# nverchev/PointCloudCounterfactual

Hardware: AMD Instinct MI355X
Metric: clouds/sec Chamfer+EMD fwd+bwd, N=2048 B=32 (higher is better)
Workload: dtype f32; 1 GPU; BASELINE configs[1]+[2]: N=2048 B=32 per GPU, nn_distance (Chamfer, mean) fwd+bwd + match_cost (approxmatch+matchcost) fwd+bwd through the autograd surface; inputs = "recon" clouds (reference permuted + N(0, 0.02^2): a trained autoencoder, SURVEY 8(d)); the 8(d) stress set (both clouds i.i.d. U[0,1]^3) is value_stress (--full); emd_mode=implicit, batch_per_gpu=32, n_points=2048, global_batch=32, parallelism=batch-sharded x1, no data-path collective, launcher=single process

## Files before the change

### include/pcc_test_hooks.h

```cpp
#ifndef PCC_TEST_HOOKS_H
#define PCC_TEST_HOOKS_H

#ifdef __cplusplus
extern "C" {
#endif
#pragma GCC visibility push(default)

int pcc_test_inject_auction_failure(void);
int pcc_test_inject_approxmatch_failure(void);

enum {
    PCC_TUNE_AM_NOCULL = 2,
    PCC_TUNE_AM_NOSPLIT = 3,
    PCC_TUNE_AM_NORESIDENT = 4,
    PCC_TUNE_EDGE_SCATTER = 5,
    PCC_TUNE_NBRSUM_SCATTER = 6,
    PCC_TUNE_AUCTION_CLUSTER = 7,
    PCC_TUNE_KNN_NOSPLIT = 8,
    PCC_TUNE_KNN_WIDE = 9
};
int pcc_test_set_tuning(int key, int value);

#pragma GCC visibility pop
#ifdef __cplusplus
}
#endif
#endif
```

### pointcloudcounterfactual_amd/_lib.py

```python

from __future__ import annotations

import ctypes
import os
from typing import Any

import torch

_HERE = os.path.dirname(os.path.abspath(__file__))
LIB_PATH = os.environ.get('PCC_LIB_OVERRIDE') or os.path.join(_HERE, 'lib', 'libpcc_structural.so')

_vp = ctypes.c_void_p
_int = ctypes.c_int

ABI: dict[str, tuple[object, list[object]]] = {
    'pcc_version': (ctypes.c_char_p, []),
    'pcc_last_error': (ctypes.c_char_p, []),
    'pcc_last_status': (_int, []),
    'pcc_profile_enable': (None, [_int]),
    'pcc_profile_reset': (None, []),
    'pcc_profile_read': (_int, [ctypes.c_char_p, ctypes.POINTER(ctypes.c_double), ctypes.POINTER(ctypes.c_int)]),
    'nndistance': (None, [_int, _int, _vp, _int, _vp, _vp, _vp, _vp, _vp, _vp]),
    'pcc_nndistance': (_int, [_int, _int, _vp, _int, _vp, _vp, _vp, _vp, _vp, _vp]),
    'nndistancegrad': (None, [_int, _int, _vp, _int, _vp, _vp, _vp, _vp, _vp, _vp, _vp, _vp]),
# ... 32 lines not shown
    'pcc_bn_relu_bwd': (_int, [_int, _int, _int, _vp, _vp, _vp, ctypes.c_float, _vp, _vp, _vp, _int, _vp, _vp, _vp, _vp]),
    'pcc_auction_forward': (_int, [_int, _int, _vp, _vp, ctypes.c_float, _int, _vp, _vp, _vp]),
    'pcc_auction_status': (_int, []),
    'pcc_auction_backward': (_int, [_int, _int, _vp, _vp, _vp, _vp, _vp, _vp]),
    'pcc_test_inject_auction_failure': (_int, []),
    'pcc_test_inject_approxmatch_failure': (_int, []),
    'pcc_test_set_tuning': (_int, [_int, _int]),
}


def _load() -> ctypes.CDLL:
    if not os.path.exists(LIB_PATH):
        raise ImportError(
            f'{LIB_PATH} is missing: the HIP extension has not been built '
            '(run `make -C pointcloudcounterfactual_amd/csrc`); there is no fallback path.'
        )
    lib = ctypes.CDLL(LIB_PATH)
    for name, (restype, argtypes) in ABI.items():
        fn = getattr(lib, name)
        fn.restype = restype
        fn.argtypes = argtypes
    return lib


lib = _load()


def check(status: int, what: str) -> None:
    if status != 0:
        msg = lib.pcc_last_error().decode() or f'HIP kernel failed : {status}'
        raise RuntimeError(f'{what}: {msg}')


def ptr(t: torch.Tensor | None, name: str, dtype: torch.dtype, device: torch.device) -> int | None:
    if t is None:
        return None
    if t.device != device or device.type != 'cuda':
        if t.device.type != 'cuda':
            raise RuntimeError(f'{name} must be a CUDA tensor')
        raise RuntimeError(f'{name} is on {t.device}, expected {device}')
    if not t.is_contiguous():
        raise RuntimeError(f'{name} must be contiguous')
    if t.dtype != dtype:
        raise RuntimeError(f'{name} must be {dtype}, found {t.dtype}')
    return t.data_ptr()


def call(fn: Any, what: str, device: torch.device, *args: Any) -> None:
    with torch.cuda.device(device):
        check(fn(*args, torch.cuda.current_stream(device).cuda_stream), what)


TUNING = {'am_nocull': 2, 'am_nosplit': 3, 'am_noresident': 4, 'edge_scatter': 5, 'nbrsum_scatter': 6,
          'auction_cluster': 7, 'knn_nosplit': 8, 'knn_wide': 9}


def set_tuning(name: str, value: int) -> None:
    if lib.pcc_test_set_tuning(TUNING[name], int(value)) != 1:
        raise RuntimeError('test hooks are not armed: set PCC_TEST_HOOKS=1 before the library is loaded')
```

### pointcloudcounterfactual_amd/csrc/approxmatch.hip

```cpp
#include "pcc_common.hpp"
#include "pcc_test_hooks.h"
#include "wave_sort.hpp"

#include <algorithm>
#include <functional>
#include <mutex>
#include <type_traits>

namespace {

using pcc::sq3;

typedef float v4f __attribute__((ext_vector_type(4)));

constexpr int kLevels = 9;
constexpr float kLog2e = 1.44269504088896340736f;

struct LevelConsts {
    float c[kLevels];
};

__host__ LevelConsts make_levels() {
    LevelConsts lc;
    float level = -16384.0f;
    for (int i = 0; i < kLevels; i++) {
        lc.c[i] = level * kLog2e;
        level *= 0.25f;
    }
    return lc;
}

__device__ __forceinline__ float fast_exp2(float x) { return __builtin_amdgcn_exp2f(x); }

enum Phase { PH_A = 0, PH_B = 1, PH_CA = 2, PH_C = 3 };

__device__ __forceinline__ float pass_a_ratio(float remL, float sum) { return remL / (1e-9f + sum); }
struct PassB {
    float ratio, remain;
};
__device__ __forceinline__ PassB pass_b(float remR, float sum) {
    const float sumr = sum * remR;
    const float consumption = __builtin_fminf(remR / (sumr + 1e-9f), 1.0f);
    return {consumption * remR, __builtin_fmaxf(0.0f, remR - sumr)};
}
__device__ __forceinline__ float pass_c_left(float remL, float ratioL, float sum) { return __builtin_fmaxf(0.0f, remL - ratioL * sum); }

constexpr int kBox = 16;
constexpr int kLiveRow = 16;
constexpr int kInfSlot = 13;
constexpr float kZeroExp = 151.f;

struct PhaseArgs {
    int n_own, n_cand, tiles, batch;
    int own_n4, cand_n4, own_nb, cand_nb;
    const float *own_soa, *cand_soa;
    const float *cand_box;
    const float *own_box16;
    const float *w0, *w1;
    long long w0_stride, w1_stride;
    float w0c;
    float c0, c1;
// ... 366 lines not shown
                const unsigned long long alive = __ballot(remain_new != 0.f);
                if (lane == 0) atomicAdd(&a.live_out[(size_t)smp * kLiveRow], (int)__popcll(alive));
            }
            if (COWN && a.mask_out && remain_new == 0.f)
                atomicAnd(&a.mask_out[(size_t)smp * kLevels * a.mask_words + (o >> 5)], ~(1u << (o & 31)));
            if (COWN && a.clist) {
                float cx = ox[0], cy = oy[0], cz = oz[0];
#pragma unroll
                for (int r = 1; r < R; r++) {
                    cx = w == r ? ox[r] : cx;
                    cy = w == r ? oy[r] : cy;
                    cz = w == r ? oz[r] : cz;
                }
                float *cl = a.clist + (size_t)smp * 5 * a.cl_n4 + tile * TQ + e;
                cl[0] = cx;
                cl[(size_t)a.cl_n4] = cy;
                cl[(size_t)2 * a.cl_n4] = cz;
                cl[(size_t)3 * a.cl_n4] = ratio_new;
                cl[(size_t)4 * a.cl_n4] = remain_new;
            }
        } else {
            const float left = pass_c_left(a.first ? a.multiL : pre_rem, pre_ratio, t0);
            a.remain[(size_t)smp * a.remain_stride + o] = left;
            if (MODE == PH_CA) a.ratio_out[(size_t)smp * a.ratio_stride + o] = pass_a_ratio(left, t1);
        }
    }
}


template <int MODE, int R, int S, int CH, int VAR, int G = 1>
__global__ __launch_bounds__(64 * S) void am_phase_kernel(PhaseArgs a) {
    __shared__ __attribute__((aligned(16))) float smem[PhaseLds<(MODE == PH_CA ? 2 : 1), R, S, CH>::floats];
    constexpr bool COWN = VAR == V_COWN;
    int smp, tile;
    const int bid = (int)blockIdx.x, nwg = (int)gridDim.x;
    if (COWN) {
        if (a.batch % 8 == 0) {
            const int per = a.batch / 8, i = bid / 8;
            smp = (bid % 8) + 8 * (i % per);
            tile = i / per;
        } else {
            smp = bid % a.batch;
            tile = bid / a.batch;
        }
        if (a.live_in && tile > 0 && tile * (64 * R / G) >= a.live_in[(size_t)smp * kLiveRow]) return;
    } else {
        const int lid = pcc::xcd_contiguous(bid, nwg);
        smp = lid / a.tiles;
        tile = lid - smp * a.tiles;
    }
    am_phase_body<MODE, R, S, CH, VAR, G>(a, smp, tile, smem);
}

constexpr int kFineS = 8;
constexpr int kFineOG = 16;
constexpr int kFineGroups = 64 / kFineOG;
constexpr int kFineQ = 4;

__device__ __forceinline__ float row_sum16(float v) {
    v += __int_as_float(__builtin_amdgcn_update_dpp(0, __float_as_int(v), 0xB1, 0xF, 0xF, true));
    v += __int_as_float(__builtin_amdgcn_update_dpp(0, __float_as_int(v), 0x4E, 0xF, 0xF, true));
    v += __int_as_float(__builtin_amdgcn_update_dpp(0, __float_as_int(v), 0x141, 0xF, 0xF, true));
    v += __int_as_float(__builtin_amdgcn_update_dpp(0, __float_as_int(v), 0x140, 0xF, 0xF, true));
    return v;
}

struct FineOwners {
    float x[kFineQ], y[kFineQ], z[kFineQ];
};
struct FineRows {
    const float *x, *y, *z, *w0, *w1;
};

__device__ __forceinline__ void fine_group_box(const float *own_box, int own_nb, int smp, int g16, float4 &lo, float4 &hi) {
    lo = make_float4(__builtin_inff(), __builtin_inff(), __builtin_inff(), 0.f);
    hi = make_float4(-__builtin_inff(), -__builtin_inff(), -__builtin_inff(), 0.f);
    if (g16 < own_nb) {
        const float4 *ob = reinterpret_cast<const float4 *>(own_box + ((size_t)smp * own_nb + g16) * 8);
        lo = ob[0];
        hi = ob[1];
    }
}

__device__ __forceinline__ float fine_box_d2(const float4 &glo, const float4 &ghi, const float *cand_box) {
    const float4 *cb = reinterpret_cast<const float4 *>(cand_box);
    const float4 lo = cb[0], hi = cb[1];
    const float dx = fmaxf(fmaxf(glo.x - hi.x, lo.x - ghi.x), 0.f);
    const float dy = fmaxf(fmaxf(glo.y - hi.y, lo.y - ghi.y), 0.f);
    const float dz = fmaxf(fmaxf(glo.z - hi.z, lo.z - ghi.z), 0.f);
    return dx * dx + dy * dy + dz * dz;
}

template <int NBLK>
__device__ __forceinline__ void fine_block_list(bool keep, bool outer_only, int tid, int tg, int tb, int w, int lane,
                                                int *wave_cnt, unsigned char (*items)[NBLK], unsigned char *need) {
    if (tid < NBLK) need[tid] = 0;
    const unsigned long long bal = __ballot(keep);
    if (lane == 0) wave_cnt[w] = __popcll(bal);
    __syncthreads();
    const int before = (w & 1) ? wave_cnt[w - 1] : 0;
    if (keep) {
        items[tg][before + __popcll(bal & ((1ull << lane) - 1ull))] = (unsigned char)(tb | (outer_only ? 128 : 0));
        need[tb] = 1;
    }
    __syncthreads();
}

template <int NW>
__device__ __forceinline__ void fine_walk(const FineRows &rows, const unsigned char *list, int nitems, int cs, int cl, float c0,
                                          float c1, const FineOwners &own, float (&s0)[kFineQ], float (&s1)[kFineQ]) {
    for (int it = cs; it < nitems; it += 2) {
        const int item = __builtin_amdgcn_readfirstlane((int)list[it]);
        const int ci = (item & 127) * kBox + cl;
        const float x = rows.x[ci], y = rows.y[ci], z = rows.z[ci];
        if (NW == 2 && (item & 128)) {
            const float wb = rows.w1[ci];
#pragma unroll
            for (int j = 0; j < kFineQ; j++) s1[j] = __builtin_fmaf(fast_exp2(c1 * sq3(x - own.x[j], y - own.y[j], z - own.z[j])), wb, s1[j]);
            continue;
        }
        const float wa = rows.w0[ci];
        float wb = 0.f;
        if (NW == 2) wb = rows.w1[ci];
#pragma unroll
        for (int j = 0; j < kFineQ; j++) {
            const float d = sq3(x - own.x[j], y - own.y[j], z - own.z[j]);
            s0[j] = __builtin_fmaf(fast_exp2(c0 * d), wa, s0[j]);
            if (NW == 2) s1[j] = __builtin_fmaf(fast_exp2(c1 * d), wb, s1[j]);
        }
    }
}

template <int NW>
__device__ __forceinline__ void fine_reduce(float (&s0)[kFineQ], float (&s1)[kFineQ], float (*red)[2][64], int cs, int cl, int og, int quad) {
#pragma unroll
    for (int j = 0; j < kFineQ; j++) {
        s0[j] = row_sum16(s0[j]);
        if (NW == 2) s1[j] = row_sum16(s1[j]);
    }
    if (cl == 0) {
#pragma unroll
        for (int j = 0; j < kFineQ; j++) {
            red[0][cs][og * kFineOG + quad * kFineQ + j] = s0[j];
            if (NW == 2) red[1][cs][og * kFineOG + quad * kFineQ + j] = s1[j];
        }
    }
}

template <int MODE, int CH>
__global__ __launch_bounds__(64 * kFineS, MODE == PH_CA ? 4 : 8) void am_fine_kernel(PhaseArgs a) {
    constexpr int T = 64 * kFineS;
    constexpr int NW = (MODE == PH_CA) ? 2 : 1;
    constexpr bool W0_CONST = (MODE == PH_A);
    constexpr int NBLK = CH / kBox;
    static_assert(kFineGroups * NBLK == T, "one (owner group, candidate block) box test per thread");
    static_assert(kFineOG == kBox && kFineOG * kFineQ == 64, "a wave = 16 candidates x 4 owner quads");
    __shared__ __attribute__((aligned(16))) float lds_c[(3 + NW) * CH];
    __shared__ float red[NW][2][64];
    __shared__ unsigned char items[kFineGroups][NBLK];
    __shared__ unsigned char need[NBLK];
    __shared__ int wave_cnt[kFineS];

    const int lid = pcc::xcd_contiguous((int)blockIdx.x, (int)gridDim.x);
    const int smp = lid / a.tiles;
    const int tile = lid - smp * a.tiles;
    const int tid = threadIdx.x, lane = tid & 63;
    const int w = __builtin_amdgcn_readfirstlane(tid >> 6);
    const int og = w & (kFineGroups - 1);
    const int cs = w / kFineGroups;
    const int cl = lane & (kBox - 1);
    const int quad = lane / kBox;
    const float *O = a.own_soa + (size_t)smp * 3 * a.own_n4;
    const float *C = a.cand_soa + (size_t)smp * 3 * a.cand_n4;
    const float *W0 = W0_CONST ? nullptr : a.w0 + (size_t)smp * a.w0_stride;
    const float *W1 = (NW == 2) ? a.w1 + (size_t)smp * a.w1_stride : nullptr;

    FineOwners own;
    float s0[kFineQ], s1[kFineQ];
#pragma unroll
    for (int j = 0; j < kFineQ; j++) {
        int o = tile * 64 + og * kFineOG + quad * kFineQ + j;
        o = o < a.n_own ? o : a.n_own - 1;
        own.x[j] = O[o];
        own.y[j] = O[a.own_n4 + o];
        own.z[j] = O[2 * a.own_n4 + o];
        s0[j] = 0.f;
        s1[j] = 0.f;
    }
    const int own_e = (tid < 64 && tile * 64 + tid < a.n_own) ? tile * 64 + tid : -1;
    float pre_rem = 0.f, pre_ratio = 0.f;
    {
        const int oe = max(own_e, 0);
        if (MODE != PH_A && !a.first) pre_rem = a.remain[(size_t)smp * a.remain_stride + oe];
        if (MODE == PH_CA || MODE == PH_C) pre_ratio = a.ratio_in[(size_t)smp * a.ratio_stride + oe];
    }
    const int tg = tid / NBLK, tb = tid - tg * NBLK;
    float4 glo, ghi;
    fine_group_box(a.own_box16, a.own_nb, smp, tile * kFineGroups + tg, glo, ghi);
    const float c0 = a.c0, c1 = a.c1, cut2 = a.cut2;
    const FineRows rows = {lds_c, lds_c + CH, lds_c + 2 * CH, lds_c + 3 * CH, lds_c + 4 * CH};

    for (int q0 = 0; q0 < a.n_cand; q0 += CH) {
        const int cnt = min(CH, a.n_cand - q0);
        const int ngroups = (cnt + 3) / 4;
        const int nblk = (ngroups + 3) / 4;
        if (q0) __syncthreads();
        bool keep = false, outer_only = false;
        if (tb < nblk) {
            const float bd2 = fine_box_d2(glo, ghi, a.cand_box + ((size_t)smp * a.cand_nb + q0 / kBox + tb) * 8);
            keep = !(bd2 > cut2);
            outer_only = NW == 2 && bd2 > a.cut2_fine;
        }
        fine_block_list<NBLK>(keep, outer_only, tid, tg, tb, w, lane, wave_cnt, items, need);
        {
            float4 *dst4 = reinterpret_cast<float4 *>(lds_c);
            const float4 *sx = reinterpret_cast<const float4 *>(C + q0);
            const float4 *sy = reinterpret_cast<const float4 *>(C + (size_t)a.cand_n4 + q0);
            const float4 *sz = reinterpret_cast<const float4 *>(C + (size_t)2 * a.cand_n4 + q0);
            static_assert(CH / 4 <= T, "one float4 group per thread and chunk");
            const int i = tid;
            if (i < nblk * 4 && need[i >> 2]) {
                float4 vx = make_float4(0.f, 0.f, 0.f, 0.f), vy = vx, vz = vx, v0 = vx, v1 = vx;
                if (i < ngroups) {
                    vx = sx[i]; vy = sy[i]; vz = sz[i];
                    v0 = W0_CONST ? make_float4(a.w0c, a.w0c, a.w0c, a.w0c) : *reinterpret_cast<const float4 *>(W0 + q0 + 4 * i);
                    if (NW == 2) v1 = *reinterpret_cast<const float4 *>(W1 + q0 + 4 * i);
                    if (W0_CONST && i * 4 + 3 >= cnt) {
                        v0.x = i * 4 + 0 < cnt ? v0.x : 0.f;
                        v0.y = i * 4 + 1 < cnt ? v0.y : 0.f;
                        v0.z = i * 4 + 2 < cnt ? v0.z : 0.f;
                        v0.w = 0.f;
                    }
                }
                dst4[i] = vx;
                dst4[CH / 4 + i] = vy;
                dst4[2 * (CH / 4) + i] = vz;
                dst4[3 * (CH / 4) + i] = v0;
                if (NW == 2) dst4[4 * (CH / 4) + i] = v1;
            }
        }
        __syncthreads();
        fine_walk<NW>(rows, items[og], wave_cnt[2 * og] + wave_cnt[2 * og + 1], cs, cl, c0, c1, own, s0, s1);
    }
    fine_reduce<NW>(s0, s1, red, cs, cl, og, quad);
    __syncthreads();
    if (own_e < 0) return;
    const float sum0 = red[0][0][tid] + red[0][1][tid];
    const float sum1 = NW == 2 ? red[NW - 1][0][tid] + red[NW - 1][1][tid] : 0.f;
    if (MODE == PH_A) {
        a.ratio_out[(size_t)smp * a.ratio_stride + own_e] = pass_a_ratio(a.multiL, sum0);
    } else if (MODE == PH_B) {
        const PassB pb = pass_b(a.first ? a.multiR : pre_rem, sum0);
        a.ratio_out[(size_t)smp * a.ratio_stride + own_e] = pb.ratio;
        a.remain_out[(size_t)smp * a.remain_stride + own_e] = pb.remain;
        if (a.live_out) {
            const unsigned long long alive = __ballot(pb.remain != 0.f);
            if (lane == 0) atomicAdd(&a.live_out[(size_t)smp * kLiveRow], (int)__popcll(alive));
            if (a.mask_out && lane == 0) {
                unsigned *mo = a.mask_out + (size_t)smp * kLevels * a.mask_words;
                if (2 * tile < a.mask_words) mo[2 * tile] = (unsigned)alive;
                if (2 * tile + 1 < a.mask_words) mo[2 * tile + 1] = (unsigned)(alive >> 32);
            }
        }
    } else {
        const float left = pass_c_left(a.first ? a.multiL : pre_rem, pre_ratio, sum0);
        a.remain[(size_t)smp * a.remain_stride + own_e] = left;
        if (MODE == PH_CA) a.ratio_out[(size_t)smp * a.ratio_stride + own_e] = pass_a_ratio(left, sum1);
    }
}

constexpr int kFpPasses = 7;
constexpr int kFpCH = 2048;
constexpr int kBarSlot = 12;
constexpr int kErrSlot = 15;

struct FinePersistArgs {
    int n, m, n4, m4, nb1, nb2, tiles;
    const float *soa1, *soa2, *box1, *box2;
    float *rem, *lv;
    float multiL, multiR;
    float c[4], cut2[4];
    int *live_cnt;
    unsigned *live_mask;
    int mask_words;
    unsigned *host_err;
    int inject;
};

__global__ __launch_bounds__(64 * kFineS) void am_fine_persist_kernel(FinePersistArgs a) {
    constexpr int T = 64 * kFineS, CH = kFpCH, NBLK = CH / kBox;
    static_assert(kFineGroups * NBLK == T, "one (owner group, candidate block) box test per thread and direction");
    __shared__ __attribute__((aligned(16))) float lds_p[2][3 * CH];
    __shared__ __attribute__((aligned(16))) float lds_w[2][CH];
    __shared__ float red[2][2][64];
    __shared__ unsigned char items[kFineGroups][NBLK];
    __shared__ unsigned char need[NBLK];
    __shared__ int wave_cnt[kFineS];

    const int lid = pcc::xcd_contiguous((int)blockIdx.x, (int)gridDim.x);
    const int smp = lid / a.tiles;
    const int tile = lid - smp * a.tiles;
    const int tid = threadIdx.x, lane = tid & 63;
    const int w = __builtin_amdgcn_readfirstlane(tid >> 6);
    const int og = w & (kFineGroups - 1), cs = w / kFineGroups;
    const int cl = lane & (kBox - 1), quad = lane / kBox;
    const long long nm4 = (long long)a.n4 + a.m4, rs = (long long)a.n4 + 2LL * a.m4;
    const float *S1 = a.soa1 + (size_t)smp * 3 * a.n4;
    const float *S2 = a.soa2 + (size_t)smp * 3 * a.m4;
    float *LV = a.lv + (size_t)smp * kLevels * nm4;
    float *REM = a.rem + (size_t)smp * rs;
    int *row = a.live_cnt + (size_t)smp * kLiveRow;
    unsigned *bar = reinterpret_cast<unsigned *>(row + kBarSlot);
    unsigned *err = reinterpret_cast<unsigned *>(row + kErrSlot);

    for (int s = 0; s < 2; s++) {
        const float *S = s ? S2 : S1;
        const int p4 = s ? a.m4 : a.n4, ngroups = p4 / 4, nblk = (ngroups + 3) / 4;
        float4 *dst4 = reinterpret_cast<float4 *>(lds_p[s]);
        const float4 *sx = reinterpret_cast<const float4 *>(S);
        const float4 *sy = reinterpret_cast<const float4 *>(S + p4);
        const float4 *sz = reinterpret_cast<const float4 *>(S + 2 * (size_t)p4);
        for (int i = tid; i < nblk * 4; i += T) {
            float4 vx = make_float4(0.f, 0.f, 0.f, 0.f), vy = vx, vz = vx;
            if (i < ngroups) { vx = sx[i]; vy = sy[i]; vz = sz[i]; }
            dst4[i] = vx;
            dst4[CH / 4 + i] = vy;
            dst4[2 * (CH / 4) + i] = vz;
// ... 1119 lines not shown
            if (tid < off) {
                red[tid] += red[tid + off];
                red2[tid] += red2[tid + off];
            }
            __syncthreads();
        }
        if (tid == 0) f.ch_loss[smp] = f.ch_mean ? red2[0] / (float)f.ch_m + red[0] / (float)f.ch_n : red[0] + red2[0];
        return;
    }
    const bool poisoned = f.flags && (f.flags[(size_t)smp * kLiveRow + kInfSlot] | f.flags[(size_t)smp * kLiveRow + kInfSlot + 1] |
                                      f.flags[(size_t)smp * kLiveRow + kErrSlot]);
    if (which == 2) {
        if (blockIdx.x) return;
        const int parts = f.parts[2];
        float s = 0.f;
        for (int i = tid; i < parts; i += 256) s += f.part[2][(size_t)smp * parts + i];
        red[tid] = s;
        __syncthreads();
        for (int off = 128; off > 0; off >>= 1) {
            if (tid < off) red[tid] += red[tid + off];
            __syncthreads();
        }
        if (tid == 0) f.out[2][smp] = poisoned ? __builtin_nanf("") : red[0];
        return;
    }
    if (!f.out[which]) return;
    const int npts = f.npts[which], pitch = f.pitch[which], parts = f.parts[which];
    const int i = blockIdx.x * 256 + tid;
    if (i >= npts * 3) return;
    const int s = i / 3, c = i - s * 3;
    const float *p = f.part[which] + (size_t)smp * parts * pitch * 3 + i;
    const int pt = f.perm[which][(size_t)smp * npts + s];
    const size_t stride = (size_t)pitch * 3;
    float acc = p[0];
    int t = 1;
    for (; t + 8 <= parts; t += 8) {
        float v[8];
#pragma unroll
        for (int u = 0; u < 8; u++) v[u] = p[(size_t)(t + u) * stride];
#pragma unroll
        for (int u = 0; u < 8; u++) acc += v[u];
    }
    {
        float v[7];
#pragma unroll
        for (int u = 0; u < 7; u++) v[u] = p[(size_t)min(t + u, parts - 1) * stride];
#pragma unroll
        for (int u = 0; u < 7; u++)
            if (t + u < parts) acc += v[u];
    }
    f.out[which][((size_t)smp * npts + pt) * 3 + c] = poisoned ? __builtin_nanf("") : f.scale ? acc * f.scale[smp] : acc;
}

constexpr int kPhCH = 2048;
constexpr int kClistCH = 1024;

static bool cull_enabled() {
    return pcc::tuning(PCC_TUNE_AM_NOCULL) == 0;
}

template <int MODE>
const char *phase_name(int level) {
    static const char *const names[4][kLevels] = {
        {"am_phase_kernel<A> L0", "", "", "", "", "", "", "", ""},
        {"am_phase_kernel<B> L0", "am_phase_kernel<B> L1", "am_phase_kernel<B> L2", "am_phase_kernel<B> L3",
         "am_phase_kernel<B> L4", "am_phase_kernel<B> L5", "am_phase_kernel<B> L6", "am_phase_kernel<B> L7",
         "am_phase_kernel<B> L8"},
        {"am_phase_kernel<CA> L0", "am_phase_kernel<CA> L1", "am_phase_kernel<CA> L2", "am_phase_kernel<CA> L3",
         "am_phase_kernel<CA> L4", "am_phase_kernel<CA> L5", "am_phase_kernel<CA> L6", "am_phase_kernel<CA> L7", ""},
        {"", "", "", "", "", "", "", "", "am_phase_kernel<C> L8"}};
    return names[MODE][level];
}

template <int MODE, int R, int S, int G = 1>
int launch_phase_rs(PhaseArgs a, int b, int var, hipStream_t st, const char *what) {
    a.tiles = pcc::ceil_div(a.n_own, 64 * R / G);
    a.batch = b;
    const long long grid = (long long)b * a.tiles;
    if (grid > 0x7fffffffLL) return pcc::invalid("approxmatch: grid too large");
    {
        pcc::ProfScope prof(phase_name<MODE>(a.level), st);
        const dim3 g((unsigned)grid), blk(64 * S);
        if (var == V_CLIST && (MODE == PH_CA || MODE == PH_C))
            hipLaunchKernelGGL((am_phase_kernel<(MODE == PH_CA || MODE == PH_C) ? MODE : PH_C, R, S, kClistCH, V_CLIST>), g, blk, 0, st, a);
        else if (var == V_COWN && MODE == PH_B)
            hipLaunchKernelGGL((am_phase_kernel<PH_B, (G > 1 ? 1 : R), S, kPhCH, V_COWN, G>), g, blk, 0, st, a);
        else hipLaunchKernelGGL((am_phase_kernel<MODE, R, S, kPhCH, V_PLAIN>), g, blk, 0, st, a);
    }
    return pcc::check_launch(what);
}

template <int MODE>
int launch_fine(PhaseArgs a, int b, hipStream_t st, const char *what) {
    a.tiles = pcc::ceil_div(a.n_own, 64);
    a.batch = b;
    const long long grid = (long long)b * a.tiles;
    if (grid > 0x7fffffffLL) return pcc::invalid("approxmatch: grid too large");
    {
        pcc::ProfScope prof(phase_name<MODE>(a.level), st);
        hipLaunchKernelGGL((am_fine_kernel<(MODE == PH_C ? PH_CA : MODE), kPhCH>), dim3((unsigned)grid), dim3(64 * kFineS), 0, st, a);
    }
    return pcc::check_launch(what);
}

template <int MODE>
int launch_phase(const PhaseArgs &a, int b, int var, hipStream_t st, const char *what) {
    if (var == V_CULL) return launch_fine<MODE>(a, b, st, what);
// ... 157 lines not shown
            if (s && hipStreamWaitEvent(s, ev, 0) == hipSuccess) side = s;
        }
        (void)hipEventDestroy(ev);
    }
    ~ForkJoin() {
        if (!side) return;
        hipEvent_t ev;
        if (hipEventCreateWithFlags(&ev, hipEventDisableTiming) != hipSuccess) {
            (void)hipStreamSynchronize(side);
            return;
        }
        (void)hipEventRecord(ev, side);
        (void)hipStreamWaitEvent(main, ev, 0);
        (void)hipEventDestroy(ev);
    }
};

static bool resident_enabled() {
    return pcc::tuning(PCC_TUNE_AM_NORESIDENT) == 0;
}
int launch_fine_resident(const Sched &sc, int bc, hipStream_t st) {
    if (!sc.skip || !sc.live_cnt || !sc.live_mask || !resident_enabled()) return -1;
    if (sc.n > kFpCH || sc.m > kFpCH || sc.n < 1 || sc.m < 1) return -1;
    const int tiles = pcc::ceil_div(std::max(sc.n, sc.m), 64);
    FinePersistArgs a{};
    a.n = sc.n; a.m = sc.m; a.n4 = sc.n4; a.m4 = sc.m4; a.nb1 = sc.nb1; a.nb2 = sc.nb2; a.tiles = tiles;
    a.soa1 = sc.soa1; a.soa2 = sc.soa2; a.box1 = sc.box1; a.box2 = sc.box2;
    a.rem = sc.rem; a.lv = sc.lv; a.multiL = sc.multiL; a.multiR = sc.multiR;
    for (int i = 0; i < 4; i++) {
        a.c[i] = sc.lc.c[i];
        a.cut2[i] = zero_cut2(sc.lc, i);
    }
    a.live_cnt = sc.live_cnt;
    a.live_mask = sc.live_mask;
    a.mask_words = mask_words(sc.m4);
    static const int per_cu = [] {
        int r = 0;
        const void *k = reinterpret_cast<const void *>(am_fine_persist_kernel);
        if (hipOccupancyMaxActiveBlocksPerMultiprocessor(&r, k, 64 * kFineS, 0) != hipSuccess) (void)hipGetLastError();
        return r;
    }();
    if (per_cu < 2 || (long long)bc * tiles > pcc::device_cus()) return -1;
    pcc::CoresidentGate gate(pcc::kFineResident, st);
    if (!gate.ok) return -1;
    a.host_err = gate.sticky;
    a.inject = gate.inject;
    {
        pcc::ProfScope prof("am_fine_persist_kernel", st);
        hipLaunchKernelGGL(am_fine_persist_kernel, dim3((unsigned)(bc * tiles)), dim3(64 * kFineS), 0, st, a);
    }
    return pcc::check_launch("approxmatch(resident fine levels)");
}

Sched lane_sched(const WsLayout &L, const WsView &v, const LevelConsts &lc) {
    Sched sc{};
    sc.n = L.n; sc.m = L.m; sc.n4 = L.n4; sc.m4 = L.m4; sc.nb1 = L.nb1; sc.nb2 = L.nb2;
    sc.soa1 = v.soa1; sc.soa2 = v.soa2; sc.box1 = v.box1; sc.box2 = v.box2; sc.rem = v.rem; sc.lv = v.lv;
    if (L.n >= L.m) { sc.multiL = 1; sc.multiR = (float)(L.n / L.m); }
    else { sc.multiL = (float)(L.m / L.n); sc.multiR = 1; }
    sc.skip = cull_enabled() ? 1 : 0;
    sc.lc = lc;
    sc.clist = v.clist; sc.clist_cnt = v.clist_cnt;
    if (sc.skip) { sc.live_cnt = v.live_cnt; sc.live_mask = v.live_mask; }
    return sc;
}

int run_levels(const WsLayout &L, char *base, const float *xyz1, const float *xyz2, const LevelConsts &lc, hipStream_t st,
               const std::function<int(int, int, hipStream_t)> &lane_tail = nullptr,
               const std::function<int(int, int, hipStream_t)> &after_sort = nullptr) {
    if (const unsigned fw = pcc::take_coresident_failure(pcc::kFineResident)) {
        char buf[320];
        std::snprintf(buf, sizeof buf, "approxmatch: an earlier call on this device did not complete (a sample barrier of the resident "
                      "fine-level launch timed out: barrier %u of sample %u saw %u arrivals; the implicit path reported NaN for those "
                      "samples); this call was not started", (fw >> 4) & 0xfu, fw >> 20, (fw >> 8) & 0xfffu);
        return pcc::invalid(buf);
    }
    const bool split_enabled = pcc::tuning(PCC_TUNE_AM_NOSPLIT) == 0;

    struct Lane {
        int s0, bc;
        hipStream_t st;
        WsView v;
        Sched sc;
    };
    Lane lanes[kMaxLanes];
    int nlanes = 1;
    bool fork = false;
    if (split_enabled && L.b >= 8 && (long long)L.b * std::max(L.n, L.m) >= 32768) {
        fork = !pcc::capturing(st);
    }
    ForkJoin fj(st, fork);
    if (fj.side) nlanes = 2;
    for (int l = 0; l < nlanes; l++) {
        Lane &ln = lanes[l];
        ln.s0 = (int)((long long)L.b * l / nlanes);
        ln.bc = (int)((long long)L.b * (l + 1) / nlanes) - ln.s0;
        ln.st = l == 0 ? st : fj.side;
        ln.v = L.view(base, ln.s0);
        ln.sc = lane_sched(L, ln.v, lc);
    }
    int rc = PCC_OK;
    auto enqueue_head = [&](int l) -> int {
        const Lane &ln = lanes[l];
        const size_t s0 = (size_t)ln.s0;
        int r = sort_clouds(L, ln.v, ln.bc, xyz1 + s0 * L.n * 3, xyz2 + s0 * L.m * 3, (bool)after_sort, ln.st);
        if (!r && after_sort && l % 2 == 0) r = after_sort(ln.s0, ln.bc, ln.st);
        return r;
    };
    auto enqueue_pass = [&](int l, int p) -> int {
        const Lane &ln = lanes[l];
        int mode, var;
        const PhaseArgs a = build_phase(ln.sc, p, &mode, &var);
        switch (mode) {
        case PH_A: return launch_phase<PH_A>(a, ln.bc, var, ln.st, "approxmatch(A)");
        case PH_B: return launch_phase<PH_B>(a, ln.bc, var, ln.st, "approxmatch(B)");
        case PH_CA: return launch_phase<PH_CA>(a, ln.bc, var, ln.st, "approxmatch(CA)");
        default: return launch_phase<PH_C>(a, ln.bc, var, ln.st, "approxmatch(C)");
        }
    };
    int first_pass[kMaxLanes] = {};
    {
        for (int l = 0; l < nlanes && !rc; l++) rc = enqueue_head(l);
        if (rc) return rc;
        {
            pcc::ProfScope seq0("am_phase_sequence", lanes[0].st, true);
            pcc::ProfScope seq1("am_phase_sequence", lanes[nlanes > 1 ? 1 : 0].st, true, nlanes >= 2);
            for (int l = 0; l < nlanes && !rc; l++) {
                const int r = launch_fine_resident(lanes[l].sc, lanes[l].bc, lanes[l].st);
                if (r > 0) rc = r;
                else if (r == 0) first_pass[l] = kFpPasses;
            }
            for (int p = 0; p < sched_phases() && !rc; p++)
                for (int l = 0; l < nlanes && !rc; l++)
                    if (p >= first_pass[l]) rc = enqueue_pass(l, p);
            if (rc) return rc;
        }
        if (after_sort)
            for (int l = 1; l < nlanes; l += 2)
                if (int rc2 = after_sort(lanes[l].s0, lanes[l].bc, lanes[l].st)) return rc2;
        if (lane_tail) {
            for (int l = 0; l < nlanes; l++)
                if (int rc2 = lane_tail(lanes[l].s0, lanes[l].bc, lanes[l].st)) return rc2;
        }
    }
    return PCC_OK;
}

int approxmatch_impl(int b, int n, int m, const float *xyz1, const float *xyz2, float *match, float *temp,
                     void *workspace, size_t workspace_bytes, float *cost_out, hipStream_t st) {
    const WsLayout L(b, n, m);
    if (workspace_bytes < L.total) return pcc::invalid("approxmatch: workspace too small");
    if (!aligned16(workspace)) return pcc::invalid("approxmatch: workspace must be 16-byte aligned");
    char *base = static_cast<char *>(workspace);
    const LevelConsts lc = make_levels();
    int rc = run_levels(L, base, xyz1, xyz2, lc, st);
    if (rc) return rc;
    const WsView v = L.view(base, 0);
    hipLaunchKernelGGL(am_unpermute_kernel, dim3(pcc::ceil_div(n + m, 256), b), dim3(256), 0, st, n, m, L.n4, L.m4, v.lv, v.rem,
                       v.rank1, v.rank2, v.live_cnt, v.lv_orig, temp);
    rc = pcc::check_launch("approxmatch(unpermute)");
    if (rc) return rc;
    const dim3 grid(pcc::ceil_div(n, kMatKT), pcc::ceil_div(m, kMatLT), b);
    const bool vec = (n % 4 == 0) && aligned16(match);
    if (cost_out) {
        {
            pcc::ProfScope prof("am_materialise_kernel<cost>", st);
            if (vec) hipLaunchKernelGGL((am_materialise_kernel<true, true>), grid, dim3(256), 0, st, n, m, xyz1, xyz2, v.lv_orig, lc, match, v.cpart);
            else hipLaunchKernelGGL((am_materialise_kernel<true, false>), grid, dim3(256), 0, st, n, m, xyz1, xyz2, v.lv_orig, lc, match, v.cpart);
        }
        rc = pcc::check_launch("approxmatch(materialise+cost)");
        if (rc) return rc;
        hipLaunchKernelGGL(reduce_rows_kernel, dim3(b), dim3(256), 0, st, (int)cost_parts(n, m), v.cpart, cost_out);
        return pcc::check_launch("approxmatch(cost reduce)");
    }
    {
        pcc::ProfScope prof("am_materialise_kernel", st);
        if (vec) hipLaunchKernelGGL((am_materialise_kernel<false, true>), grid, dim3(256), 0, st, n, m, xyz1, xyz2, v.lv_orig, lc, match, nullptr);
        else hipLaunchKernelGGL((am_materialise_kernel<false, false>), grid, dim3(256), 0, st, n, m, xyz1, xyz2, v.lv_orig, lc, match, nullptr);
    }
    return pcc::check_launch("approxmatch(materialise)");
}
// ... 248 lines not shown
```

### pointcloudcounterfactual_amd/csrc/pcc_common.cpp

```cpp
#include "pcc_common.hpp"

#include <atomic>
#include <cstdlib>
#include <mutex>
#include <string>
#include <utility>
#include <vector>

namespace {
thread_local int t_status = 0;
thread_local char t_msg[320] = "";
}

namespace {
int g_tuning[16] = {};
}

namespace pcc {
int device_cus() {
    static std::atomic<int> cache[64];
    int dev = 0;
    if (hipGetDevice(&dev) != hipSuccess || dev < 0 || dev >= 64) return 0;
    int v = cache[dev].load(std::memory_order_relaxed);
    if (v == 0) {
// ... 136 lines not shown

namespace pcc {
bool capturing(hipStream_t st) {
    hipStreamCaptureStatus cap = hipStreamCaptureStatusNone;
    if (hipStreamIsCapturing(st, &cap) != hipSuccess) (void)hipGetLastError();
    return cap != hipStreamCaptureStatusNone;
}

struct CoresidentDevice {
    unsigned *host = nullptr, *mapped = nullptr;
    hipEvent_t last = nullptr;
    hipStream_t last_stream = nullptr;
    bool inject[kCoresidentKinds] = {}, tried = false;
};
namespace {
std::mutex g_coresident_mu;
CoresidentDevice *coresident_device() {
    static CoresidentDevice devs[64];
    int dev = 0;
    if (hipGetDevice(&dev) != hipSuccess || dev < 0 || dev >= 64) return nullptr;
    CoresidentDevice &d = devs[dev];
    if (!std::exchange(d.tried, true)) {
        void *h = nullptr, *p = nullptr;
        if (hipHostMalloc(&h, kCoresidentKinds * sizeof(unsigned), hipHostMallocMapped) == hipSuccess &&
            hipHostGetDevicePointer(&p, h, 0) == hipSuccess && hipEventCreateWithFlags(&d.last, hipEventDisableTiming) == hipSuccess) {
            d.host = static_cast<unsigned *>(std::memset(h, 0, kCoresidentKinds * sizeof(unsigned)));
            d.mapped = static_cast<unsigned *>(p);
        } else {
            (void)hipGetLastError();
        }
    }
    return d.host ? &d : nullptr;
}
}

CoresidentGate::CoresidentGate(CoresidentKind kind, hipStream_t s) : st(s) {
    if (capturing(st)) return;
    g_coresident_mu.lock();
    if (!(dev = coresident_device())) {
        g_coresident_mu.unlock();
        return;
    }
    if (dev->last_stream && dev->last_stream != st) (void)hipStreamWaitEvent(st, dev->last, 0);
    ok = true;
    sticky = dev->mapped + kind;
    inject = std::exchange(dev->inject[kind], false);
}
CoresidentGate::~CoresidentGate() {
    if (!dev) return;
    if (hipEventRecord(dev->last, st) == hipSuccess) dev->last_stream = st;
    g_coresident_mu.unlock();
}

unsigned take_coresident_failure(CoresidentKind kind) {
    std::lock_guard<std::mutex> lk(g_coresident_mu);
    CoresidentDevice *d = coresident_device();
    return d ? __atomic_exchange_n(&d->host[kind], 0u, __ATOMIC_RELAXED) : 0;
}
}

#include "pcc_test_hooks.h"
static bool hooks_armed() {
    static const bool armed = [] {
        const char *e = std::getenv("PCC_TEST_HOOKS");
        return e && e[0] == '1';
    }();
    return armed;
}
extern "C" int pcc_test_set_tuning(int key, int value) {
    if (!hooks_armed() || key < 0 || key >= 16) return 0;
    __atomic_store_n(&g_tuning[key], value, __ATOMIC_RELAXED);
    return 1;
}
static int inject_failure(pcc::CoresidentKind kind) {
    if (!hooks_armed()) return 0;
    std::lock_guard<std::mutex> lk(pcc::g_coresident_mu);
    pcc::CoresidentDevice *d = pcc::coresident_device();
    if (d) d->inject[kind] = true;
    return d ? 1 : 0;
}
extern "C" int pcc_test_inject_auction_failure(void) { return inject_failure(pcc::kAuctionCluster); }
extern "C" int pcc_test_inject_approxmatch_failure(void) { return inject_failure(pcc::kFineResident); }
```

### pointcloudcounterfactual_amd/csrc/pcc_common.hpp

```cpp
#pragma once
#include <hip/hip_runtime.h>

#include <cstdio>
#include <cstring>

#include "pcc_structural.h"

#if defined(__HIP_DEVICE_COMPILE__) && !defined(__gfx950__)
#error "libpcc_structural is written for gfx950 (MI355X) only"
#endif

namespace pcc {

constexpr int kWave = 64;

void set_error(int status, const char *what);
void clear_error();

inline int check_launch(const char *what) {
    hipError_t err = hipGetLastError();
    if (err != hipSuccess) {
        char buf[256];
        std::snprintf(buf, sizeof buf, "HIP kernel failed : %d (%s) in %s", (int)err, hipGetErrorString(err), what);
        set_error((int)err, buf);
// ... 66 lines not shown
};
int match_cost_with_chamfer(int b, int n, int m, const float *xyz1, const float *xyz2, float *cost, float *grad1,
                            float *grad2, hipStream_t st, const ChamferOut &chamfer);

__device__ __forceinline__ int xcd_contiguous(int bid, int nwg) {
    if (nwg <= 8) return bid;
    const int q = nwg / 8, r = nwg % 8, x = bid % 8;
    return (x < r ? x * (q + 1) : r * (q + 1) + (x - r) * q) + bid / 8;
}

constexpr int kSortBox = 16;
int sort_cloud_cmajor(int b, int c, int n, const float *x, float4 *aos, float *box16, int *perm, hipStream_t st);

int knn_wide(int b, int c, int n, int k, const float *x, int64_t *indices, hipStream_t st);

void launch_sqnorm(int b, int c, int n, const float *x, float *sq, hipStream_t st);

bool capturing(hipStream_t st);

template <class T>
__device__ __forceinline__ T agent_ld(const T *p) { return __hip_atomic_load(p, __ATOMIC_RELAXED, __HIP_MEMORY_SCOPE_AGENT); }
template <class T>
__device__ __forceinline__ void agent_st(T *p, T v) { __hip_atomic_store(p, v, __ATOMIC_RELAXED, __HIP_MEMORY_SCOPE_AGENT); }

__device__ __forceinline__ void coresident_fail(unsigned *err, unsigned *host_err, unsigned code) {
    const unsigned was = __hip_atomic_exchange(err, 1u, __ATOMIC_RELAXED, __HIP_MEMORY_SCOPE_AGENT);
    unsigned expected = 0;
    if (host_err && !was)
        __hip_atomic_compare_exchange_strong(host_err, &expected, code, __ATOMIC_RELAXED, __ATOMIC_RELAXED, __HIP_MEMORY_SCOPE_SYSTEM);
}

template <int SLEEP, unsigned BOUND, class Code>
__device__ __forceinline__ bool coresident_barrier(unsigned *ctr, unsigned target, unsigned *err, unsigned *host_err, Code code) {
    asm volatile("s_waitcnt vmcnt(0)" ::: "memory");
    __syncthreads();
    __shared__ int failed;
    if (threadIdx.x == 0) {
        failed = 0;
        __hip_atomic_fetch_add(ctr, 1u, __ATOMIC_RELAXED, __HIP_MEMORY_SCOPE_AGENT);
        unsigned spins = 0;
        while (agent_ld(ctr) < target) {
            __builtin_amdgcn_s_sleep(SLEEP);
            if (++spins > BOUND || agent_ld(err)) {
                coresident_fail(err, host_err, code());
                failed = 1;
                break;
            }
        }
    }
    __syncthreads();
    return failed == 0;
}

enum CoresidentKind { kAuctionCluster = 0, kFineResident = 1, kCoresidentKinds = 2 };

struct CoresidentGate {
    CoresidentGate(CoresidentKind kind, hipStream_t st);
    ~CoresidentGate();
    bool ok = false, inject = false;
    unsigned *sticky = nullptr;
    struct CoresidentDevice *dev = nullptr;
    hipStream_t st;
};

unsigned take_coresident_failure(CoresidentKind kind);

}
```

Baseline: 70520 clouds/s.

## Chain approxmatch fine-level passes in one ticketed launch with per-sample progress waits

Adds a fallback path used when the resident fine-level launch is unavailable. It fuses the seven fine-level passes into a single kernel where blocks take work units in order from an atomic ticket and wait on per-sample progress counters before reading the previous pass's results. This replaces separate kernel launches and their full-grid boundaries with fine-grained dependency waits, so later-pass tiles can start while other samples are still finishing. The cost is spin-waiting, agent-scope atomics and fences, and timeout error handling that relies on blocks being scheduled in ticket order.

Measured after the change: 53000 clouds/s, median of 2. -24.8%, worse.

```diff
diff --git a/include/pcc_test_hooks.h b/include/pcc_test_hooks.h
--- a/include/pcc_test_hooks.h
+++ b/include/pcc_test_hooks.h
@@ -17,7 +17,8 @@
     PCC_TUNE_NBRSUM_SCATTER = 6,
     PCC_TUNE_AUCTION_CLUSTER = 7,
     PCC_TUNE_KNN_NOSPLIT = 8,
-    PCC_TUNE_KNN_WIDE = 9
+    PCC_TUNE_KNN_WIDE = 9,
+    PCC_TUNE_AM_NOCHAIN = 10
 };
 int pcc_test_set_tuning(int key, int value);
 
diff --git a/pointcloudcounterfactual_amd/_lib.py b/pointcloudcounterfactual_amd/_lib.py
--- a/pointcloudcounterfactual_amd/_lib.py
+++ b/pointcloudcounterfactual_amd/_lib.py
@@ -108,7 +108,7 @@
 
 
 TUNING = {'am_nocull': 2, 'am_nosplit': 3, 'am_noresident': 4, 'edge_scatter': 5, 'nbrsum_scatter': 6,
-          'auction_cluster': 7, 'knn_nosplit': 8, 'knn_wide': 9}
+          'auction_cluster': 7, 'knn_nosplit': 8, 'knn_wide': 9, 'am_nochain': 10}
 
 
 def set_tuning(name: str, value: int) -> None:
diff --git a/pointcloudcounterfactual_amd/csrc/approxmatch.hip b/pointcloudcounterfactual_amd/csrc/approxmatch.hip
--- a/pointcloudcounterfactual_amd/csrc/approxmatch.hip
+++ b/pointcloudcounterfactual_amd/csrc/approxmatch.hip
@@ -7,6 +7,12 @@
 #include <mutex>
 #include <type_traits>
 
+#ifndef CHAIN_SLEEP
+#define CHAIN_SLEEP 1
+#endif
+#ifndef CHAIN_PERSIST
+#define CHAIN_PERSIST 0
+#endif
 namespace {
 
 using pcc::sq3;
@@ -479,6 +485,7 @@
     am_phase_body<MODE, R, S, CH, VAR, G>(a, smp, tile, smem);
 }
 
+constexpr int kPhCH = 2048;
 constexpr int kFineS = 8;
 constexpr int kFineOG = 16;
 constexpr int kFineGroups = 64 / kFineOG;
@@ -574,23 +581,34 @@
     }
 }
 
-template <int MODE, int CH>
-__global__ __launch_bounds__(64 * kFineS, MODE == PH_CA ? 4 : 8) void am_fine_kernel(PhaseArgs a) {
+constexpr int kBarSlot = 12;
+constexpr int kErrSlot = 15;
+constexpr int kTicketSlot = 11;
+
+template <int NW, int CH>
+struct FineLds {
+    float c[(3 + NW) * CH] __attribute__((aligned(16)));
+    float red[NW][2][64];
+    unsigned char items[kFineGroups][CH / kBox];
+    unsigned char need[CH / kBox];
+    int wave_cnt[kFineS];
+};
+
+struct ChainWait {
+    unsigned *progress, *err, *host_err;
+    unsigned target, code;
+};
+
+template <int MODE, int CH, bool CHAIN, class LDS>
+__device__ __forceinline__ void am_fine_body(const PhaseArgs &a, int smp, int tile, LDS &lds, const ChainWait &cw) {
     constexpr int T = 64 * kFineS;
     constexpr int NW = (MODE == PH_CA) ? 2 : 1;
     constexpr bool W0_CONST = (MODE == PH_A);
     constexpr int NBLK = CH / kBox;
     static_assert(kFineGroups * NBLK == T, "one (owner group, candidate block) box test per thread");
     static_assert(kFineOG == kBox && kFineOG * kFineQ == 64, "a wave = 16 candidates x 4 owner quads");
-    __shared__ __attribute__((aligned(16))) float lds_c[(3 + NW) * CH];
-    __shared__ float red[NW][2][64];
-    __shared__ unsigned char items[kFineGroups][NBLK];
-    __shared__ unsigned char need[NBLK];
-    __shared__ int wave_cnt[kFineS];
-
-    const int lid = pcc::xcd_contiguous((int)blockIdx.x, (int)gridDim.x);
-    const int smp = lid / a.tiles;
-    const int tile = lid - smp * a.tiles;
+    float *lds_c = lds.c;
+
     const int tid = threadIdx.x, lane = tid & 63;
     const int w = __builtin_amdgcn_readfirstlane(tid >> 6);
     const int og = w & (kFineGroups - 1);
@@ -616,11 +634,12 @@
     }
     const int own_e = (tid < 64 && tile * 64 + tid < a.n_own) ? tile * 64 + tid : -1;
     float pre_rem = 0.f, pre_ratio = 0.f;
-    {
+    auto load_pre = [&] {
         const int oe = max(own_e, 0);
         if (MODE != PH_A && !a.first) pre_rem = a.remain[(size_t)smp * a.remain_stride + oe];
         if (MODE == PH_CA || MODE == PH_C) pre_ratio = a.ratio_in[(size_t)smp * a.ratio_stride + oe];
-    }
+    };
+    if (!CHAIN) load_pre();
     const int tg = tid / NBLK, tb = tid - tg * NBLK;
     float4 glo, ghi;
     fine_group_box(a.own_box16, a.own_nb, smp, tile * kFineGroups + tg, glo, ghi);
@@ -638,7 +657,7 @@
             keep = !(bd2 > cut2);
             outer_only = NW == 2 && bd2 > a.cut2_fine;
         }
-        fine_block_list<NBLK>(keep, outer_only, tid, tg, tb, w, lane, wave_cnt, items, need);
+        fine_block_list<NBLK>(keep, outer_only, tid, tg, tb, w, lane, lds.wave_cnt, lds.items, lds.need);
         {
             float4 *dst4 = reinterpret_cast<float4 *>(lds_c);
             const float4 *sx = reinterpret_cast<const float4 *>(C + q0);
@@ -646,10 +665,17 @@
             const float4 *sz = reinterpret_cast<const float4 *>(C + (size_t)2 * a.cand_n4 + q0);
             static_assert(CH / 4 <= T, "one float4 group per thread and chunk");
             const int i = tid;
-            if (i < nblk * 4 && need[i >> 2]) {
-                float4 vx = make_float4(0.f, 0.f, 0.f, 0.f), vy = vx, vz = vx, v0 = vx, v1 = vx;
+            const bool mine = i < nblk * 4 && lds.need[i >> 2];
+            auto stage_xyz = [&] {
+                float4 vx = make_float4(0.f, 0.f, 0.f, 0.f), vy = vx, vz = vx;
+                if (i < ngroups) { vx = sx[i]; vy = sy[i]; vz = sz[i]; }
+                dst4[i] = vx;
+                dst4[CH / 4 + i] = vy;
+                dst4[2 * (CH / 4) + i] = vz;
+            };
+            auto stage_w = [&] {
+                float4 v0 = make_float4(0.f, 0.f, 0.f, 0.f), v1 = v0;
                 if (i < ngroups) {
-                    vx = sx[i]; vy = sy[i]; vz = sz[i];
                     v0 = W0_CONST ? make_float4(a.w0c, a.w0c, a.w0c, a.w0c) : *reinterpret_cast<const float4 *>(W0 + q0 + 4 * i);
                     if (NW == 2) v1 = *reinterpret_cast<const float4 *>(W1 + q0 + 4 * i);
                     if (W0_CONST && i * 4 + 3 >= cnt) {
@@ -659,47 +685,96 @@
                         v0.w = 0.f;
                     }
                 }
-                dst4[i] = vx;
-                dst4[CH / 4 + i] = vy;
-                dst4[2 * (CH / 4) + i] = vz;
                 dst4[3 * (CH / 4) + i] = v0;
                 if (NW == 2) dst4[4 * (CH / 4) + i] = v1;
-            }
+            };
+            if (mine) stage_xyz();
+            if (CHAIN && MODE != PH_A && q0 == 0) {
+                if (!pcc::chain_wait<CHAIN_SLEEP, (1u << 22)>(cw.progress, cw.target, cw.err, cw.host_err, [&] { return cw.code; })) return;
+                load_pre();
+            }
+            if (mine) stage_w();
         }
         __syncthreads();
-        fine_walk<NW>(rows, items[og], wave_cnt[2 * og] + wave_cnt[2 * og + 1], cs, cl, c0, c1, own, s0, s1);
-    }
-    fine_reduce<NW>(s0, s1, red, cs, cl, og, quad);
+        fine_walk<NW>(rows, lds.items[og], lds.wave_cnt[2 * og] + lds.wave_cnt[2 * og + 1], cs, cl, c0, c1, own, s0, s1);
+    }
+    fine_reduce<NW>(s0, s1, lds.red, cs, cl, og, quad);
     __syncthreads();
-    if (own_e < 0) return;
-    const float sum0 = red[0][0][tid] + red[0][1][tid];
-    const float sum1 = NW == 2 ? red[NW - 1][0][tid] + red[NW - 1][1][tid] : 0.f;
-    if (MODE == PH_A) {
-        a.ratio_out[(size_t)smp * a.ratio_stride + own_e] = pass_a_ratio(a.multiL, sum0);
-    } else if (MODE == PH_B) {
-        const PassB pb = pass_b(a.first ? a.multiR : pre_rem, sum0);
-        a.ratio_out[(size_t)smp * a.ratio_stride + own_e] = pb.ratio;
-        a.remain_out[(size_t)smp * a.remain_stride + own_e] = pb.remain;
-        if (a.live_out) {
-            const unsigned long long alive = __ballot(pb.remain != 0.f);
-            if (lane == 0) atomicAdd(&a.live_out[(size_t)smp * kLiveRow], (int)__popcll(alive));
-            if (a.mask_out && lane == 0) {
-                unsigned *mo = a.mask_out + (size_t)smp * kLevels * a.mask_words;
-                if (2 * tile < a.mask_words) mo[2 * tile] = (unsigned)alive;
-                if (2 * tile + 1 < a.mask_words) mo[2 * tile + 1] = (unsigned)(alive >> 32);
-            }
-        }
-    } else {
-        const float left = pass_c_left(a.first ? a.multiL : pre_rem, pre_ratio, sum0);
-        a.remain[(size_t)smp * a.remain_stride + own_e] = left;
-        if (MODE == PH_CA) a.ratio_out[(size_t)smp * a.ratio_stride + own_e] = pass_a_ratio(left, sum1);
-    }
+    auto put = [](float *p, float v) {
+        if (CHAIN) pcc::agent_st(p, v);
+        else *p = v;
+    };
+    if (own_e >= 0) {
+        const float sum0 = lds.red[0][0][tid] + lds.red[0][1][tid];
+        const float sum1 = NW == 2 ? lds.red[NW - 1][0][tid] + lds.red[NW - 1][1][tid] : 0.f;
+        if (MODE == PH_A) {
+            put(&a.ratio_out[(size_t)smp * a.ratio_stride + own_e], pass_a_ratio(a.multiL, sum0));
+        } else if (MODE == PH_B) {
+            const PassB pb = pass_b(a.first ? a.multiR : pre_rem, sum0);
+            put(&a.ratio_out[(size_t)smp * a.ratio_stride + own_e], pb.ratio);
+            put(&a.remain_out[(size_t)smp * a.remain_stride + own_e], pb.remain);
+            if (a.live_out) {
+                const unsigned long long alive = __ballot(pb.remain != 0.f);
+                if (lane == 0) atomicAdd(&a.live_out[(size_t)smp * kLiveRow], (int)__popcll(alive));
+                if (a.mask_out && lane == 0) {
+                    unsigned *mo = a.mask_out + (size_t)smp * kLevels * a.mask_words;
+                    if (2 * tile < a.mask_words) mo[2 * tile] = (unsigned)alive;
+                    if (2 * tile + 1 < a.mask_words) mo[2 * tile + 1] = (unsigned)(alive >> 32);
+                }
+            }
+        } else {
+            const float left = pass_c_left(a.first ? a.multiL : pre_rem, pre_ratio, sum0);
+            put(&a.remain[(size_t)smp * a.remain_stride + own_e], left);
+            if (MODE == PH_CA) put(&a.ratio_out[(size_t)smp * a.ratio_stride + own_e], pass_a_ratio(left, sum1));
+        }
+    }
+    if (CHAIN) pcc::chain_arrive(cw.progress);
+}
+
+template <int MODE, int CH>
+__global__ __launch_bounds__(64 * kFineS, MODE == PH_CA ? 4 : 8) void am_fine_kernel(PhaseArgs a) {
+    __shared__ FineLds<(MODE == PH_CA ? 2 : 1), CH> lds;
+    const int lid = pcc::xcd_contiguous((int)blockIdx.x, (int)gridDim.x);
+    const int smp = lid / a.tiles;
+    am_fine_body<MODE, CH, false>(a, smp, lid - smp * a.tiles, lds, ChainWait{});
 }
 
 constexpr int kFpPasses = 7;
+struct FineChainArgs {
+    PhaseArgs p[kFpPasses];
+    unsigned unit_end[kFpPasses];
+    unsigned need[kFpPasses];
+    int *live_cnt;
+    unsigned *host_err;
+};
+static_assert(sizeof(FineChainArgs) <= 4096, "kernel arguments");
+
+__global__ __launch_bounds__(64 * kFineS, 4) void am_fine_chain_kernel(FineChainArgs c) {
+    __shared__ FineLds<2, kPhCH> lds;
+#if CHAIN_PERSIST
+    for (;;) {
+#endif
+    const unsigned t = pcc::chain_ticket(reinterpret_cast<unsigned *>(c.live_cnt + kTicketSlot));
+    if (t >= c.unit_end[kFpPasses - 1]) return;
+    int p = 0;
+#pragma unroll
+    for (int q = 0; q + 1 < kFpPasses; q++) p += t >= c.unit_end[q] ? 1 : 0;
+    const PhaseArgs &a = c.p[p];
+    const unsigned u = t - (p ? c.unit_end[p - 1] : 0u);
+    const int smp = (int)(u / (unsigned)a.tiles), tile = (int)(u - (unsigned)smp * (unsigned)a.tiles);
+    int *row = c.live_cnt + (size_t)smp * kLiveRow;
+    const ChainWait cw = {reinterpret_cast<unsigned *>(row + kBarSlot), reinterpret_cast<unsigned *>(row + kErrSlot), c.host_err,
+                          c.need[p], 1u | ((unsigned)p << 4) | (((unsigned)tile & 0xfffu) << 8) | ((unsigned)smp << 20)};
+    if (p == 0) am_fine_body<PH_A, kPhCH, true>(a, smp, tile, lds, cw);
+    else if (p & 1) am_fine_body<PH_B, kPhCH, true>(a, smp, tile, lds, cw);
+    else am_fine_body<PH_CA, kPhCH, true>(a, smp, tile, lds, cw);
+#if CHAIN_PERSIST
+    __syncthreads();
+    }
+#endif
+}
+
 constexpr int kFpCH = 2048;
-constexpr int kBarSlot = 12;
-constexpr int kErrSlot = 15;
 
 struct FinePersistArgs {
     int n, m, n4, m4, nb1, nb2, tiles;
@@ -1925,7 +2000,6 @@
     f.out[which][((size_t)smp * npts + pt) * 3 + c] = poisoned ? __builtin_nanf("") : f.scale ? acc * f.scale[smp] : acc;
 }
 
-constexpr int kPhCH = 2048;
 constexpr int kClistCH = 1024;
 
 static bool cull_enabled() {
@@ -2189,6 +2263,39 @@
     return pcc::check_launch("approxmatch(resident fine levels)");
 }
 
+static bool chain_enabled() {
+    return pcc::tuning(PCC_TUNE_AM_NOCHAIN) == 0;
+}
+int launch_fine_chain(const Sched &sc, int bc, hipStream_t st) {
+    if (!sc.skip || !sc.live_cnt || !chain_enabled()) return -1;
+    FineChainArgs c{};
+    long long units = 0, arrivals = 0;
+    for (int p = 0; p < kFpPasses; p++) {
+        int mode, var;
+        c.p[p] = build_phase(sc, p, &mode, &var);
+        if (var != V_CULL) return -1;
+        c.p[p].tiles = pcc::ceil_div(c.p[p].n_own, 64);
+        c.p[p].batch = bc;
+        c.need[p] = (unsigned)arrivals;
+        arrivals += c.p[p].tiles;
+        units += (long long)bc * c.p[p].tiles;
+        if (units > 0x7fffffffLL) return pcc::invalid("approxmatch: grid too large");
+        c.unit_end[p] = (unsigned)units;
+    }
+    c.live_cnt = sc.live_cnt;
+    if (!(c.host_err = pcc::sticky_word(pcc::kFineChain))) return -1;
+    {
+        pcc::ProfScope prof("am_fine_chain_kernel", st);
+#if CHAIN_PERSIST
+        const long long slots = (long long)CHAIN_PERSIST * std::max(pcc::device_cus(), 1);
+        hipLaunchKernelGGL(am_fine_chain_kernel, dim3((unsigned)std::min(units, slots)), dim3(64 * kFineS), 0, st, c);
+#else
+        hipLaunchKernelGGL(am_fine_chain_kernel, dim3((unsigned)units), dim3(64 * kFineS), 0, st, c);
+#endif
+    }
+    return pcc::check_launch("approxmatch(chained fine levels)");
+}
+
 Sched lane_sched(const WsLayout &L, const WsView &v, const LevelConsts &lc) {
     Sched sc{};
     sc.n = L.n; sc.m = L.m; sc.n4 = L.n4; sc.m4 = L.m4; sc.nb1 = L.nb1; sc.nb2 = L.nb2;
@@ -2210,6 +2317,13 @@
         std::snprintf(buf, sizeof buf, "approxmatch: an earlier call on this device did not complete (a sample barrier of the resident "
                       "fine-level launch timed out: barrier %u of sample %u saw %u arrivals; the implicit path reported NaN for those "
                       "samples); this call was not started", (fw >> 4) & 0xfu, fw >> 20, (fw >> 8) & 0xfffu);
+        return pcc::invalid(buf);
+    }
+    if (const unsigned fw = pcc::take_coresident_failure(pcc::kFineChain)) {
+        char buf[320];
+        std::snprintf(buf, sizeof buf, "approxmatch: an earlier call on this device did not complete (a unit of the chained "
+                      "fine-level launch timed out waiting for the passes before it: pass %u, tile %u of sample %u; the implicit path "
+                      "reported NaN for those samples); this call was not started", (fw >> 4) & 0xfu, (fw >> 8) & 0xfffu, fw >> 20);
         return pcc::invalid(buf);
     }
     const bool split_enabled = pcc::tuning(PCC_TUNE_AM_NOSPLIT) == 0;
@@ -2263,7 +2377,8 @@
             pcc::ProfScope seq0("am_phase_sequence", lanes[0].st, true);
             pcc::ProfScope seq1("am_phase_sequence", lanes[nlanes > 1 ? 1 : 0].st, true, nlanes >= 2);
             for (int l = 0; l < nlanes && !rc; l++) {
-                const int r = launch_fine_resident(lanes[l].sc, lanes[l].bc, lanes[l].st);
+                int r = launch_fine_resident(lanes[l].sc, lanes[l].bc, lanes[l].st);
+                if (r < 0) r = launch_fine_chain(lanes[l].sc, lanes[l].bc, lanes[l].st);
                 if (r > 0) rc = r;
                 else if (r == 0) first_pass[l] = kFpPasses;
             }
diff --git a/pointcloudcounterfactual_amd/csrc/pcc_common.cpp b/pointcloudcounterfactual_amd/csrc/pcc_common.cpp
--- a/pointcloudcounterfactual_amd/csrc/pcc_common.cpp
+++ b/pointcloudcounterfactual_amd/csrc/pcc_common.cpp
@@ -212,6 +212,12 @@
     g_coresident_mu.unlock();
 }
 
+unsigned *sticky_word(CoresidentKind kind) {
+    std::lock_guard<std::mutex> lk(g_coresident_mu);
+    CoresidentDevice *d = coresident_device();
+    return d ? d->mapped + kind : nullptr;
+}
+
 unsigned take_coresident_failure(CoresidentKind kind) {
     std::lock_guard<std::mutex> lk(g_coresident_mu);
     CoresidentDevice *d = coresident_device();
diff --git a/pointcloudcounterfactual_amd/csrc/pcc_common.hpp b/pointcloudcounterfactual_amd/csrc/pcc_common.hpp
--- a/pointcloudcounterfactual_amd/csrc/pcc_common.hpp
+++ b/pointcloudcounterfactual_amd/csrc/pcc_common.hpp
@@ -142,7 +142,41 @@
     return failed == 0;
 }
 
-enum CoresidentKind { kAuctionCluster = 0, kFineResident = 1, kCoresidentKinds = 2 };
+__device__ __forceinline__ unsigned chain_ticket(unsigned *ticket_word) {
+    __shared__ unsigned ticket;
+    if (threadIdx.x == 0) ticket = __hip_atomic_fetch_add(ticket_word, 1u, __ATOMIC_RELAXED, __HIP_MEMORY_SCOPE_AGENT);
+    __syncthreads();
+    return ticket;
+}
+
+template <int SLEEP, unsigned BOUND, class Code>
+__device__ __forceinline__ bool chain_wait(unsigned *progress, unsigned target, unsigned *err, unsigned *host_err, Code code) {
+    __shared__ int failed;
+    if (threadIdx.x == 0) {
+        failed = 0;
+        unsigned spins = 0;
+        while (agent_ld(progress) < target) {
+            __builtin_amdgcn_s_sleep(SLEEP);
+            if (++spins > BOUND || agent_ld(err)) {
+                coresident_fail(err, host_err, code());
+                failed = 1;
+                break;
+            }
+        }
+        __builtin_amdgcn_fence(__ATOMIC_ACQUIRE, "agent");
+        asm volatile("s_waitcnt vmcnt(0)" ::: "memory");
+    }
+    __syncthreads();
+    return failed == 0;
+}
+
+__device__ __forceinline__ void chain_arrive(unsigned *progress) {
+    asm volatile("s_waitcnt vmcnt(0)" ::: "memory");
+    __syncthreads();
+    if (threadIdx.x == 0) __hip_atomic_fetch_add(progress, 1u, __ATOMIC_RELAXED, __HIP_MEMORY_SCOPE_AGENT);
+}
+
+enum CoresidentKind { kAuctionCluster = 0, kFineResident = 1, kFineChain = 2, kCoresidentKinds = 3 };
 
 struct CoresidentGate {
     CoresidentGate(CoresidentKind kind, hipStream_t st);
@@ -155,4 +189,6 @@
 
 unsigned take_coresident_failure(CoresidentKind kind);
 
+unsigned *sticky_word(CoresidentKind kind);
+
 }
```
